# OHDSI/bayes-bridge

Measured on AMD Instinct MI355X. Metric: Gibbs iters/sec (cg sampler), higher is better.
Workload: dtype f64

## Files before the change

### bayes-bridge_amd/bayesbridge_amd/_lib.py

```python
import ctypes
import os
from ctypes import (POINTER, byref, c_char_p, c_double, c_int, c_int32,
                    c_int64, c_uint64, c_void_p)

_HERE = os.path.dirname(os.path.abspath(__file__))
LIB_PATH = os.path.join(os.path.dirname(_HERE), "libbbx.so")

ABI_VERSION = 113
FORMAT_AUTO, FORMAT_CSR, FORMAT_TILED = 0, 1, 2
F64, F32 = 0, 1
MODEL_LINEAR, MODEL_LOGIT = 0, 1
MODEL_PROBIT = 2
MODEL_STUDENT_T = 3
MODEL_CENSORED = 4
PRED_LINEAR, PRED_LOGIT, PRED_POISSON = 0, 1, 2
GSCALE_SAMPLE, GSCALE_OPTIMIZE, GSCALE_FIXED = 0, 1, 2
BATCH_ALLOW_SLOW = 1
ERR_NUMERIC = -4
COX_FAMILIES = ("cox", "coxcp", "coxef", "coxw", "coxfg")
SAMPLER_CG, SAMPLER_CHOLESKY, SAMPLER_WOODBURY = 0, 1, 2
STREAM_ETA1, STREAM_ETA2 = 1, 2

_lib = None
finalizing = False
# ... 131 lines not shown
        "bbx_chain_get_summary": (
            [hp, c_void_p, c_void_p, POINTER(c_int64)], c_int),
        "bbx_chain_init_obs_prec": ([hp], c_int),
        "bbx_chain_get_iteration": ([hp, POINTER(c_int64)], c_int),
        "bbx_chain_set_iteration": ([hp, c_int64], c_int),
        "bbx_chain_get_seed": ([hp, POINTER(c_uint64)], c_int),
        "bbx_chain_set_seed": ([hp, c_uint64], c_int),
        "bbx_chain_set_gscale_update": ([hp, c_int], c_int),
        "bbx_chain_set_coef_sampler": ([hp, c_int], c_int),
        "bbx_chol_release": ([hp], c_int),
        "bbx_chain_eta": ([hp, c_int64, c_void_p, c_void_p], c_int),
        "bbx_chain_get_logp": (
            [hp, POINTER(c_double), POINTER(c_double)], c_int),
        "bbx_chain_get_latent": ([hp, c_void_p], c_int),
        "bbx_chain_get_zbase": ([hp, c_void_p], c_int),
        "bbx_chain_set_df": ([hp, c_double], c_int),
        "bbx_chain_get_df": ([hp, POINTER(c_double)], c_int),
        "bbx_chain_run": (
            [hp, c_int, c_int, c_int, c_int, c_double, c_void_p, c_void_p,
             c_void_p, c_void_p, c_void_p, c_void_p], c_int),
        "bbx_chain_set_progress": ([hp, c_int, c_void_p, c_void_p], c_int),
        "bbx_chain_run_host": (
            [hp, c_int, c_int, c_int, c_int, c_double, c_void_p, c_void_p,
             c_void_p, c_void_p, c_void_p, c_void_p], c_int),
        "bbx_batch_create": ([hp, c_int, c_void_p, POINTER(hp)], c_int),
        "bbx_batch_create_opts": (
            [hp, c_int, c_void_p, ctypes.c_uint, POINTER(hp)], c_int),
        "bbx_batch_predict": ([hp, c_int, POINTER(c_double)], c_int),
        "bbx_batch_unconverged": ([hp, POINTER(c_int)], c_int),
        "bbx_batch_destroy": ([hp], c_int),
# ... 199 lines not shown
```

### bayes-bridge_amd/bayesbridge_amd/design_matrix.py

```python
import ctypes
import warnings
from ctypes import byref, c_double, c_int, c_int64, c_void_p

import numpy as np
import scipy.sparse as sparse

from . import _lib


def _ptr(a):
    return None if a is None else a.ctypes.data_as(c_void_p)


def remove_intercept_indicator(X):
    n_rows = X.shape[0]
    if sparse.issparse(X):
        first = np.asarray(X.mean(axis=0)).ravel()
        second = np.asarray(X.multiply(X).mean(axis=0)).ravel()
        variance = second - first ** 2
    else:
        variance = np.var(X, axis=0)
    constant = variance < n_rows * 2. ** -52
    if constant.any():
        warnings.warn(
# ... 84 lines not shown
        return (int(a.value), int(b.value)), (pa.value, pb.value)

    @property
    def cg_launches(self):
        from ctypes import c_int
        v = c_int()
        _lib.check(self._lib.bbx_design_cg_launches(self._h, byref(v)))
        return int(v.value)

    def cg_stats(self, reset=False):
        from ctypes import c_int64
        a, b, c = c_int64(), c_int64(), c_int64()
        _lib.check(self._lib.bbx_design_cg_stats(
            self._h, byref(a), byref(b), byref(c), 1 if reset else 0))
        return int(a.value), int(b.value), int(c.value)

    def set_cg_fold(self, on):
        _lib.check(self._lib.bbx_design_set_cg_fold(
            self._h, -1 if on is None else int(bool(on))))

    @property
    def fused_operator_bytes(self):
        v = c_int64()
        _lib.check(self._lib.bbx_design_fused_operator_bytes(self._h,
                                                              byref(v)))
        return int(v.value)

    def tiled_info(self, chains=1):
        out = {}
        base = {1: 0, 2: 2, 4: 4}[int(chains)]
# ... 331 lines not shown
```

### bayes-bridge_amd/bayesbridge_amd/device_chain.py

```python
from ctypes import byref, c_double, c_int64, c_uint64, c_void_p

import numpy as np

from . import _lib

_GSCALE_MODES = {'sample': _lib.GSCALE_SAMPLE, 'optimize': _lib.GSCALE_OPTIMIZE,
                 None: _lib.GSCALE_FIXED}


_MODEL_CODES = {'linear': _lib.MODEL_LINEAR, 'logit': _lib.MODEL_LOGIT,
                'probit': _lib.MODEL_PROBIT,
                'student_t': _lib.MODEL_STUDENT_T,
                'censored': _lib.MODEL_CENSORED}


def _ptr(a):
    return None if a is None else a.ctypes.data_as(c_void_p)


def _f64(a):
    return np.ascontiguousarray(a, dtype=np.float64)


class HipGibbsChain():
# ... 105 lines not shown
        df = float(df)
        if not (df > 0. and np.isfinite(df)):
            raise ValueError("df must be finite and positive: %r" % df)
        _lib.check(self._lib.bbx_chain_set_df(self._c, df))

    def get_df(self):
        df = c_double()
        _lib.check(self._lib.bbx_chain_get_df(self._c, byref(df)))
        return float(df.value)

    def get_zbase(self):
        out = np.empty(self.P)
        _lib.check(self._lib.bbx_chain_get_zbase(self._c, _ptr(out)))
        return out

    def init_obs_prec(self):
        _lib.check(self._lib.bbx_chain_init_obs_prec(self._c))

    def set_summary(self, mean, square, n_averaged):
        mean, square = _f64(mean), _f64(square)
        if mean.shape != (self.P,) or square.shape != (self.P,):
            raise ValueError("summaries must have length %d" % self.P)
        _lib.check(self._lib.bbx_chain_set_summary(
            self._c, _ptr(mean), _ptr(square), int(n_averaged)))

    def get_summary(self):
        mean, square, n_avg = np.empty(self.P), np.empty(self.P), c_int64()
        _lib.check(self._lib.bbx_chain_get_summary(
            self._c, _ptr(mean), _ptr(square), byref(n_avg)))
        return mean, square, int(n_avg.value)
# ... 197 lines not shown
```

### bayes-bridge_amd/csrc/api.hip

```cpp
#include <algorithm>
#include <cmath>
#include <cstring>
#include <new>

#include <fcntl.h>
#include <sys/file.h>
#include <unistd.h>

#include <condition_variable>
#include <mutex>
#include <thread>
#include <unordered_set>

#include "common.hpp"
#include "tiled_layout.hpp"

namespace bbx {

static thread_local std::string g_last_error;

void set_error(const std::string& msg) { g_last_error = msg; }
int fail(int code, const std::string& msg) {
  g_last_error = msg;
  return code;
// ... 1379 lines not shown

uint64_t bbx_launch_count(void) {
  return bbx::g_launch_count.load(std::memory_order_relaxed);
}

int bbx_design_cg_stats(bbx_design* h, int64_t* solves, int64_t* empty_launches,
                        int64_t* naps, int reset) {
  BBX_TRY(check_handle(h));
  if (solves) *solves = h->cg_solves;
  if (empty_launches) *empty_launches = h->cg_empty_launches;
  if (naps) *naps = h->cg_naps;
  if (reset) h->cg_solves = h->cg_empty_launches = h->cg_naps = 0;
  return BBX_OK;
}

int bbx_design_cg_launches(const bbx_design* h, int* per_iteration) {
  BBX_TRY(check_handle(h));
  if (!per_iteration) return fail(BBX_ERR_INVALID, "per_iteration is NULL");
  int n = 5;
  if (tiled_fold_applies(h)) {
    n = 3;
  } else if (!h->sparse && dense_fused_applies(h)) {
    n = 3;
  } else if (h->sparse && h->format == BBX_FORMAT_TILED) {
    int G = 0;
    if (!h->hybrid && tiled_describe(h, 0, nullptr, nullptr, nullptr, &G,
                                     nullptr, nullptr) == BBX_OK && G == 1)
      n = 4;
  }
  *per_iteration = n;
// ... 17 lines not shown
```

### bayes-bridge_amd/csrc/cg_sampler.hip

```cpp
#include <sys/prctl.h>
#include <time.h>

#include "common.hpp"
#include "philox.hpp"
#include "tiled_layout.hpp"

namespace bbx {

int launch_cg_setup(bbx_design* h, int n_unshrunk, const double* phi,
                    const double* sd, const double* x0, double* s, double* d,
                    double* xs, CGState* st, double atol);
int launch_cg_direction(bbx_design* h, int k, CGState* st,
                        const double* rr_part, const double* r, double* pvec,
                        const double* s, double* sp, double* c_part,
                        const double* d = nullptr, double* pdp_part = nullptr,
                        unsigned long long* word = nullptr,
                        unsigned long long tag = 0);
int launch_cg_update(bbx_design* h, int k, CGState* st, const double* pq_part,
                     const double* pvec, const double* q, double* x, double* r,
                     double* rr_part);
int launch_cg_finish(bbx_design* h, const double* s, const double* x,
                     double* coef);

__global__ __launch_bounds__(256) void fill_normal_kernel(
    int64_t len, uint64_t seed, uint64_t stream, double* __restrict__ out,
    int prio) {
  if (prio) __builtin_amdgcn_s_setprio(3);
  for (int64_t i = (int64_t)blockIdx.x * blockDim.x + threadIdx.x; i < len;
       i += (int64_t)gridDim.x * blockDim.x) {
    Philox g(seed, stream, (uint64_t)i);
    out[i] = g.normal();
  }
// ... 95 lines not shown
  double* sp = h->w_P[6].as<double>() + (h->intercept ? 1 : 0);
  CGState* st = h->cg_state.as<CGState>();
  const bool fold = tiled_fold_applies(h);
  double* sr = h->w_P[9].as<double>() + (h->intercept ? 1 : 0);
  double* tu = h->w_n[2].as<double>();

  if (d_eta1 == nullptr) {
    double* e1 = h->w_n[2].as<double>();
    double* e2 = h->w_P[8].as<double>();
    BBX_TRY(launch_fill_normal(h, h->n, seed, STREAM_ETA1, e1));
    BBX_TRY(launch_fill_normal(h, h->P, seed, STREAM_ETA2, e2));
    d_eta1 = e1;
    d_eta2 = e2;
  }

  BBX_TRY(launch_cg_setup(h, n_unshrunk, d_phi, d_sd, d_x0, s, d, x, st, atol));

  CGState* host_st = static_cast<CGState*>(h->host_pinned);
  if (x0_zero < 0) {
    int* d_flag = &st->pad;
    int* h_flag = reinterpret_cast<int*>(host_st);
    BBX_HIP(hipMemsetAsync(d_flag, 0, sizeof(int), h->stream));
    BBX_LAUNCH(any_nonzero_kernel, dim3(NPART), dim3(256), 0,
                       h->stream, h->P, d_x0, d_flag);
    BBX_HIP(hipGetLastError());
    BBX_HIP(hipMemcpyAsync(h_flag, d_flag, sizeof(int), hipMemcpyDeviceToHost,
                           h->stream));
    BBX_HIP(hipStreamSynchronize(h->stream));
    x0_zero = (*h_flag == 0) ? 1 : 0;
  }

// ... 1 lines not shown
    double* w = h->w_n[1].as<double>();
    TdotEpilogue ep;
    ep.mode = TD_RESID;
    ep.s = s;
    ep.d = d;
    ep.x = x0_zero ? nullptr : x;
    ep.z = d_z;
    ep.phi = d_phi;
    ep.eta2 = d_eta2;
    ep.dot_part = part_slot(h, PS_RR);
    if (fold) {
      ep.fold_sr = sr;
      ep.fold_cr_part = part_slot(h, PS_C);
    }
    if (!x0_zero && !h->sparse && dense_fused_applies(h)) {
      BBX_TRY(launch_prep_v(h, x, s, sp, part_slot(h, PS_C)));
      BBX_TRY(launch_sqrt_scale(h, d_omega, d_eta1, w, part_slot(h, PS_SUMW),
                                nullptr, true));
      const int st_f =
          launch_operator_dense_fused(h, sp, d_omega, ep, r, nullptr, w);
      if (st_f != 0)
        return st_f < 0 ? st_f
                        : fail(BBX_ERR_STATE,
                               "single-pass dense operator refused its design");
    } else {
      const double* t0 = nullptr;
      if (!x0_zero) {
        double* t = h->w_n[0].as<double>();
        BBX_TRY(launch_prep_v(h, x, s, sp, part_slot(h, PS_C)));
        BBX_TRY(launch_dot(h, sp, d_omega, t, nullptr));
        t0 = t;
      }
      BBX_TRY(launch_sqrt_scale(h, d_omega, d_eta1, w, part_slot(h, PS_SUMW),
                                t0, t0 == nullptr));
      BBX_TRY(launch_tdot(h, w, part_slot(h, PS_SUMW), ep, r));
    }
  }


  struct SkipScope {
    bbx_design* h;
    ~SkipScope() { h->skip_flag = nullptr; }
  } skip_scope{h};
  h->skip_flag = &st->done;
// ... 44 lines not shown
    ep.dot_part = part_slot(h, PS_RR);
    ep.cg_x = x;
    ep.cg_r = r;
    ep.cg_state = st;
    ep.cg_k = kk;
    ep.pdp_part = pdp;
    ep.twt_part = part_slot(h, PS_TWT);
    ep.fold_sr = sr;
    ep.fold_cr_part = part_slot(h, PS_C);
    BBX_TRY(launch_tdot(h, h->w_n[0].as<double>(), part_slot(h, PS_SUMW), ep, q));
    return timer_end(h, 2);
  };
  auto iteration = [&](int kk) -> int {
    if (fold) return folded_iteration(kk);
    BBX_TRY(launch_cg_direction(h, kk, st, part_slot(h, PS_RR), r, pvec, s, sp,
                                part_slot(h, PS_C), d, pdp, word, tag));
    return operator_and_update(kk);
  };
  static const int ahead_env = getenv("BBX_CG_AHEAD") ? atoi(getenv("BBX_CG_AHEAD")) : 0;
  const int ahead = ahead_env >= 1 ? (ahead_env < 64 ? ahead_env : 64)
                    : h->n >= 50000 ? 1 : h->n >= 10000 ? 2 : 4;
  int free_run = 0;
  if (h->cg_recent_n > 0) {
    free_run = h->cg_recent[0];
    for (int i = 1; i < h->cg_recent_n; ++i)
      free_run = h->cg_recent[i] < free_run ? h->cg_recent[i] : free_run;
    free_run -= 1;
  }
  if (free_run > maxiter) free_run = maxiter;
  static const int sleep_env = getenv("BBX_CG_SLEEP") ? atoi(getenv("BBX_CG_SLEEP")) : -1;
  static const bool sleep_on = sleep_env >= 0 ? sleep_env != 0 : cores_per_rank() < 3;
// ... 55 lines not shown
        h->cg_naps += 1;
      }
      slept = true;
      continue;
    }
    if (++spins > (1u << 14)) {
      const hipError_t qe = hipStreamQuery(h->stream);
      if (qe != hipSuccess && qe != hipErrorNotReady) BBX_HIP(qe);
      spins = 0;
    }
    __builtin_ia32_pause();
  }
  h->timer.cur_tag = -1;
  h->tail_ran = false;
  h->coef_in_flight = false;
  BBX_TRY(launch_cg_finish(h, s, x, d_coef));
  if (done) {
    if (!h->ev_poll)
      BBX_HIP(hipEventCreateWithFlags(&h->ev_poll, hipEventDisableTiming));
    BBX_HIP(hipEventRecord(h->ev_poll, h->stream));
    h->coef_in_flight = true;
    if (h->tail_hook) {
      const bool timing = h->timer.enabled;
      h->timer.enabled = false;
      h->skip_flag = nullptr;
      const int rc = h->tail_hook(h->tail_ctx);
      h->timer.enabled = timing;
      if (rc < 0) return rc;
      h->tail_ran = true;
    }
  } else {
// ... 32 lines not shown
```

### bayes-bridge_amd/csrc/chain.hip

```cpp
#include <cmath>
#include <new>
#include <string>
#include <vector>

#include "chain.hpp"
#include "philox.hpp"
#include "samplers.hpp"
#include "pg_queue.hpp"

namespace bbx {

__device__ inline double wsum(double x) { return wave_allsum(x); }

__device__ inline double block_total_256(double x) {
  __shared__ double s_w[256 / WAVE];
  x = wsum(x);
  if ((threadIdx.x & (WAVE - 1)) == 0) s_w[threadIdx.x / WAVE] = x;
  __syncthreads();
  double r = 0.;
  if (threadIdx.x == 0)
    for (int k = 0; k < 256 / WAVE; ++k) r += s_w[k];
  __syncthreads();
  return r;
}

__device__ inline double shrunk_scale(double gscale, double lscale,
                                      double slab) {
  const double raw = gscale * lscale;
  const double ratio = raw / slab;
  return raw / sqrt(1. + ratio * ratio);
}

__global__ __launch_bounds__(256) void chain_prior_kernel(
    int64_t P, int nu, int model, double slab, long long n_avg,
    const ChainScalars* __restrict__ sc, const double* __restrict__ lscale,
    const double* __restrict__ sd_unshrunk, const double* __restrict__ mean,
    const double* __restrict__ square, const double* __restrict__ zbase,
    double* __restrict__ phi, double* __restrict__ x0, double* __restrict__ sd,
    double* __restrict__ z, int store_idx, double* __restrict__ samp_gs,
    double* __restrict__ samp_lp) {
  const double g = sc->gscale;
  const double zs =
      (model == BBX_MODEL_LINEAR || model == BBX_MODEL_CENSORED) ? sc->obs_prec
                                                                 : 1.;
  if (store_idx >= 0 && blockIdx.x == 0 && threadIdx.x == 0) {
    samp_gs[store_idx] = g;
    samp_lp[store_idx] = sc->logp();
  }
  for (int64_t j = (int64_t)blockIdx.x * 256 + threadIdx.x; j < P;
       j += (int64_t)gridDim.x * 256) {
    double prior_sd, guess = mean[j];
    if (j < nu) {
      prior_sd = sd_unshrunk[j];
    } else {
      prior_sd = shrunk_scale(g, lscale[j - nu], slab);
      guess *= prior_sd;
    }
    phi[j] = 1. / prior_sd;
    x0[j] = guess;
    double est = 1.;
    if (n_avg > 1) {
      const double k = (double)n_avg;
      const double m = mean[j];
      const double var = k / (k - 1.) * (square[j] - m * m);
      const double w = (k - 1.) / (k - 1. + 5.);
      est = sqrt(w * var + (1. - w) * 1.);
    }
    sd[j] = est;
    z[j] = zs * zbase[j];
  }
}

#define BBX_BRANCH_PRIO() do { if (prio) __builtin_amdgcn_s_setprio(3); } while (0)
static int lscale_prio() {
  static const int on = getenv("BBX_LSCALE_PRIO") ? atoi(getenv("BBX_LSCALE_PRIO")) : 1;
  return on;
}
static int branch_prio() {
  static const int on = !(getenv("BBX_BRANCH_PRIO") && atoi(getenv("BBX_BRANCH_PRIO")) == 0);
  return on;
}
__global__ __launch_bounds__(256) void chain_summary_kernel(
    int64_t P, int nu, double slab, long long n_avg,
    const ChainScalars* __restrict__ sc, const double* __restrict__ lscale,
// ... 485 lines not shown
  if (!on || !h->sparse || h->format != BBX_FORMAT_TILED || h->hybrid) return false;
  int G = 0;
  return tiled_describe(h, 0, nullptr, nullptr, nullptr, &G, nullptr, nullptr) ==
             BBX_OK && G == 1;
}

static int chain_check(const bbx_chain* c) {
  if (!c || !c->h) return fail(BBX_ERR_INVALID, "chain handle is NULL");
  return BBX_OK;
}

static double power_exp_ave_magnitude(double exponent) {
  return std::tgamma(2. / exponent) / std::tgamma(1. / exponent);
}

int chain_pre_draw(bbx_chain* c) {
  bbx_design* h = c->h;
  hipStream_t s = h->stream;
  const int64_t P = h->P, n = h->n;
  ChainScalars* sc = c->scalars.as<ChainScalars>();
  BBX_LAUNCH(chain_prior_kernel, dim3(NPART), dim3(256), 0, s, P,
                     c->n_unshrunk, c->model, c->slab,
                     (long long)c->n_averaged, sc, c->lscale.as<double>(),
                     c->sd_unshrunk.as<double>(), c->mean.as<double>(),
                     c->square.as<double>(), c->zbase.as<double>(),
                     c->phi.as<double>(), c->x0.as<double>(),
                     c->sd.as<double>(), c->z.as<double>(), c->pending_store,
                     c->samp_gscale.as<double>(), c->samp_logp.as<double>());
  c->pending_store = -1;
  if (c->model == BBX_MODEL_LINEAR || c->model == BBX_MODEL_CENSORED)
    BBX_LAUNCH(chain_fill_obs_prec_kernel, dim3(grid_for(n, ROW_GRID)),
                       dim3(256), 0, s, n, sc, c->obs_prec.as<double>());
  BBX_HIP(hipGetLastError());
  return BBX_OK;
}

int chain_post_draw(bbx_chain* c, bool have_psi, int phases,
                    bbx_chain* branch_of) {
  bbx_design* h = c->h;
  hipStream_t s = h->stream;
  const int64_t P = h->P, n = h->n;
  const int nu = c->n_unshrunk;
  const int64_t n_shrunk = P - nu;
  ChainScalars* sc = c->scalars.as<ChainScalars>();
// ... 112 lines not shown

  launch_err = hipGetLastError();
  if (phases & POST_JOIN) {
    if (fork) {
      BBX_HIP(hipEventRecord(c->ev_join, s_b));
      BBX_HIP(hipStreamWaitEvent(s, c->ev_join, 0));
    }
    c->iter += 1;
  }
  BBX_HIP(launch_err);
  return BBX_OK;
}

static int chain_step(bbx_chain* c, int maxiter, double atol, int* n_cg_iter) {
  const uint64_t it = (uint64_t)c->iter;
  BBX_TRY(chain_pre_draw(c));
  int info = 0;
  const bool have_eta = c->eta_iter == (long long)it && c->eta1_next.ptr;
  if (c->coef_sampler == BBX_SAMPLER_CHOLESKY) {
    bbx_design* h = c->h;
    if (!have_eta) {
      if (!c->eta2_next.ptr)
        BBX_TRY(c->eta2_next.alloc(sizeof(double) * (size_t)h->P));
      BBX_TRY(launch_fill_normal(h, h->P, cg_draw_seed(c, it), STREAM_ETA2,
                                 c->eta2_next.as<double>()));
    }
    const bool linear = c->model == BBX_MODEL_LINEAR ||
                        c->model == BBX_MODEL_CENSORED;
    const bool probit = c->model == BBX_MODEL_PROBIT;
    const int st = chol_sample_device(
        h, linear || probit ? nullptr : c->obs_prec.as<double>(), 1.,
// ... 32 lines not shown
        linear || probit ? 0 : 1, c->eta1_next.as<double>(), c->eta2_next.as<double>(),
        c->coef.as<double>());
    c->eta_iter = -1;
    if (st < 0) return st;
    c->coef_sample = nullptr;
    if (n_cg_iter) *n_cg_iter = 0;
    BBX_TRY(chain_post_draw(c, false, POST_ALL));
    return 0;
  }
  struct TailScope {
    bbx_design* h;
    ~TailScope() {
      h->tail_hook = nullptr;
      h->tail_ctx = nullptr;
      h->coef_copy = nullptr;
    }
  } tail_scope{c->h};
  c->h->coef_copy = c->coef_sample;
  if (chain_tail_applies(c)) {
    c->h->tail_hook = chain_tail_hook;
    c->h->tail_ctx = c;
  }

  int st = cg_sample_device(
      c->h, c->obs_prec.as<double>(), c->phi.as<double>(), c->z.as<double>(),
      c->x0.as<double>(), c->sd.as<double>(), c->n_unshrunk,
      have_eta ? c->eta1_next.as<double>() : nullptr,
      have_eta ? c->eta2_next.as<double>() : nullptr,
      cg_draw_seed(c, it), maxiter, atol, c->coef.as<double>(), n_cg_iter,
      &info, c->mean_zero ? 1 : 0);
  c->eta_iter = -1;
  if (st < 0) return st;
  c->mean_zero = false;
// ... 500 lines not shown
      return fail(BBX_ERR_INVALID, "bbx_chain_get_df: not a student_t chain");
    if (!df) return fail(BBX_ERR_INVALID, "bbx_chain_get_df: df is NULL");
    *df = c->df;
    return BBX_OK;
  });
}

int bbx_chain_get_zbase(bbx_chain* c, double* out) {
  return no_throw([&]() -> int {
    BBX_TRY(chain_check(c));
    if (!out) return fail(BBX_ERR_INVALID, "bbx_chain_get_zbase: out is NULL");
    BBX_HIP(hipSetDevice(c->h->device));
    BBX_HIP(hipStreamSynchronize(c->h->stream));
    BBX_HIP(hipMemcpy(out, c->zbase.ptr, sizeof(double) * (size_t)c->h->P,
                      hipMemcpyDeviceToHost));
    return BBX_OK;
  });
}

int bbx_chain_init_obs_prec(bbx_chain* c) {
  BBX_TRY(chain_check(c));
  bbx_design* h = c->h;
  BBX_HIP(hipSetDevice(h->device));
  if (c->model == BBX_MODEL_PROBIT) return chain_probit_refresh(c);
  BBX_TRY(chain_linear_predictor(c));
  const int rg = grid_for(h->n, ROW_GRID);
  if (c->model == BBX_MODEL_STUDENT_T) {
    double* rp = c->row_part.as<double>();
    BBX_LAUNCH(chain_rss_kernel, dim3(rg), dim3(256), 0, h->stream, h->n,
               c->outcome.as<double>(), c->psi.as<double>(), rp);
// ... 302 lines not shown
```

### bayes-bridge_amd/csrc/chain.hpp

```cpp
#pragma once
#include <cmath>

#include "common.hpp"

namespace bbx {

constexpr int ROW_GRID = 2048;

struct alignas(128) ChainScalars {
  double gscale;
  double logprior;
  double abs_pow_sum;
  long long n_gscale_clamped;
  long long n_lscale_fixed;
  alignas(128) double obs_prec;
  double loglik;
  __host__ __device__ double logp() const { return loglik + logprior; }
};

}

struct bbx_chain {
  bbx_design* h = nullptr;
  int model = BBX_MODEL_LOGIT;
// ... 23 lines not shown
  long long eta_iter = -1;
  bbx::DevMem samp_gscale, samp_logp;
  int pending_store = -1;
  double* coef_sample = nullptr;
  void* pinned = nullptr;
  hipStream_t stream2 = nullptr;
  hipEvent_t ev_join = nullptr;
};

namespace bbx {

inline uint64_t cg_draw_seed(const bbx_chain* c, uint64_t it) {
  return c->seed + 0x9E3779B97F4A7C15ull * (it + 1);
}

int chain_pre_draw(bbx_chain* c);
enum { POST_BRANCH = 1, POST_MAIN = 2, POST_JOIN = 4, POST_ALL = 7 };
int chain_post_draw(bbx_chain* c, bool have_psi, int phases,
                    bbx_chain* branch_of = nullptr);
int chain_begin_run(bbx_chain* c, int n_sample);
int chain_save_sample(bbx_chain* c, int idx, double* d_coef, double* d_lscale,
                      double* d_obs_prec);
int chain_end_run(bbx_chain* c, int n_sample, double* gscale, double* logp);

int launch_chain_probit(bbx_chain* c, uint64_t stream, int* row_blocks);
int launch_sumw_fold(bbx_design* h, const double* block_sums, int count);

int launch_student_t_tau(bbx_chain* c, uint64_t stream);
int launch_student_t_mix(bbx_chain* c, uint64_t stream, int* row_blocks);
int launch_student_t_finish(bbx_chain* c, int row_blocks);
double student_t_row_const(double nu);
// ... 5 lines not shown
```

### bayes-bridge_amd/csrc/common.hpp

```cpp
#pragma once

#include <hip/hip_runtime.h>
#include <stdint.h>

#include <exception>
#include <new>
#include <string>
#include <vector>

#include "../../include/bbx.h"

#include <atomic>
namespace bbx {
extern std::atomic<unsigned long long> g_launch_count;
}
#define BBX_LAUNCH(...)                                                   \
  do {                                                                    \
    bbx::g_launch_count.fetch_add(1, std::memory_order_relaxed);          \
    hipLaunchKernelGGL(__VA_ARGS__);                                      \
  } while (0)
#define BBX_LAUNCH_EXT(...)                                               \
  do {                                                                    \
    bbx::g_launch_count.fetch_add(1, std::memory_order_relaxed);          \
    hipExtLaunchKernelGGL(__VA_ARGS__);                                   \
// ... 97 lines not shown
  }
};

struct CGState {
  double rho[2];
  double atol;
  double bnorm2;
  int n_iter;
  int done;
  int bad;
  int pad;
  int running;
  int pad2;
};

struct KernelTimer {
  bool enabled = false;
  int period = 1;
  static constexpr int FAMILIES = 3;
  int64_t seen[FAMILIES] = {0, 0, 0};
  bool armed[FAMILIES] = {false, false, false};
  struct Pair {
    hipEvent_t a, b;
    int tag;
  };
  std::vector<Pair> pending[FAMILIES];
  std::vector<Pair> pool;
  int cur_tag = -1;
  std::vector<float> samples[FAMILIES];
};
// ... 50 lines not shown

  int64_t n_dot = 0, n_tdot = 0;
  int last_cg_iter = 0;
  unsigned long long* cg_word_host = nullptr;
  unsigned long long* cg_word_dev = nullptr;
  unsigned long long cg_serial = 0;
  int cg_recent[8] = {0, 0, 0, 0, 0, 0, 0, 0};
  int cg_recent_n = 0;
  int64_t cg_period_ns = 0;
  bool coef_in_flight = false;
  int64_t cg_empty_launches = 0, cg_solves = 0, cg_naps = 0;
  double* coef_copy = nullptr;
  int (*tail_hook)(void*) = nullptr;
  void* tail_ctx = nullptr;
  bool tail_ran = false;
  hipEvent_t ev_poll = nullptr;
  bool in_operator = false;
  uint64_t operator_serial = 0;
  int cg_fold = -1;
  const int* skip_flag = nullptr;
  bbx::KernelTimer timer;
};

namespace bbx {

enum PartSlot {
  PS_C = 0,
  PS_SUMW = 1,
  PS_PQ = 2,
  PS_RR = 3,
// ... 204 lines not shown
```

### bayes-bridge_amd/csrc/vecops.hip

```cpp
#include "common.hpp"

namespace bbx {

std::atomic<unsigned long long> g_launch_count{0};


__device__ inline double wave_sum_v(double x) { return wave_allsum(x); }

__device__ inline void block_store_partial(double x, double* part) {
  __shared__ double s_w[VEC_BLOCK / WAVE];
  x = wave_sum_v(x);
  if ((threadIdx.x & (WAVE - 1)) == 0) s_w[threadIdx.x / WAVE] = x;
  __syncthreads();
  if (threadIdx.x == 0) {
    double r = 0.;
#pragma unroll
    for (int k = 0; k < VEC_BLOCK / WAVE; ++k) r += s_w[k];
    part[blockIdx.x] = r;
  }
  __syncthreads();
}

__device__ inline double sum_partials_v(const double* part) {
  __shared__ double s_tot;
// ... 127 lines not shown
    const double sj = (jj < n_unshrunk) ? 2. * sd[jj] : 1. / ph;
    const double sp = sj * ph;
    s[jj] = sj;
    d[jj] = sp * sp;
    xs[jj] = x0[jj] / sj;
  }
}

__global__ __launch_bounds__(VEC_BLOCK) void cg_direction_kernel(
    int64_t P, int intercept, int k, CGState* __restrict__ st,
    const double* __restrict__ rr_part, const double* __restrict__ r,
    double* __restrict__ pvec, const double* __restrict__ s,
    const double* __restrict__ offset, double* __restrict__ sp,
    double* __restrict__ c_part, const double* __restrict__ d,
    double* __restrict__ pdp_part, unsigned long long* word,
    unsigned long long tag) {
  const PartLoad pl = part_issue(rr_part);
  const int64_t stride = (int64_t)gridDim.x * VEC_BLOCK;
  const int64_t j0 = (int64_t)blockIdx.x * VEC_BLOCK + threadIdx.x;
  const bool has0 = j0 < P;
  double r0 = 0., p0 = 0., s0 = 0., o0 = 0., d0 = 0.;
  if (has0) {
    r0 = r[j0];
    if (k > 0) p0 = pvec[j0];
    s0 = s[j0];
    if (j0 >= intercept) o0 = offset[j0 - intercept];
    if (pdp_part) d0 = d[j0];
  }
  const int was_done = st->done;
  const double atol = st->atol;
  const double rho_prev = (k > 0) ? st->rho[(k - 1) & 1] : 1.;
  if (was_done) return;
  const double rho = part_finish(pl);
  const bool finite = (rho == rho) && (rho - rho == 0.);
  if (!finite || sqrt(rho) < atol) {
    if (blockIdx.x == 0 && threadIdx.x == 0) {
      st->done = 1;
      st->running = 0;
      if (!finite) st->bad = 1;
      if (word)
        cg_word_store(word, tag | CG_WORD_DONE | (finite ? 0ull : CG_WORD_BAD) |
                                (unsigned long long)k);
    }
    return;
  }
  if (word && blockIdx.x == 0 && threadIdx.x == 0)
    cg_word_store(word, tag | (unsigned long long)(k + 1));
  const double beta = (k > 0) ? rho / rho_prev : 0.;
  double acc = 0., acc_d = 0.;
  if (has0) {
    double pj = r0;
    if (k > 0) pj += beta * p0;
    pvec[j0] = pj;
    const double v = s0 * pj;
    sp[j0] = v;
    if (j0 >= intercept) acc += o0 * v;
    acc_d += d0 * pj * pj;
// ... 63 lines not shown

int launch_cg_setup(bbx_design* h, int n_unshrunk, const double* phi,
                    const double* sd, const double* x0, double* s, double* d,
                    double* xs, CGState* st, double atol) {
  BBX_LAUNCH(cg_setup_kernel, dim3(NPART), dim3(VEC_BLOCK), 0,
                     h->stream, h->P, n_unshrunk, phi, sd, x0, s, d, xs, st,
                     atol);
  BBX_HIP(hipGetLastError());
  return BBX_OK;
}

int launch_cg_direction(bbx_design* h, int k, CGState* st,
                        const double* rr_part, const double* r, double* pvec,
                        const double* s, double* sp, double* c_part,
                        const double* d, double* pdp_part,
                        unsigned long long* word, unsigned long long tag) {
  BBX_LAUNCH(cg_direction_kernel, dim3(NPART), dim3(VEC_BLOCK), 0,
                     h->stream, h->P, h->intercept, k, st, rr_part, r, pvec, s,
                     h->offset.as<double>(), sp, c_part, d, pdp_part, word, tag);
  BBX_HIP(hipGetLastError());
  return BBX_OK;
}

int launch_cg_update(bbx_design* h, int k, CGState* st, const double* pq_part,
                     const double* pvec, const double* q, double* x, double* r,
                     double* rr_part) {
  BBX_LAUNCH(cg_update_kernel, dim3(NPART), dim3(VEC_BLOCK), 0,
                     h->stream, h->P, k, st, pq_part, pvec, q, x, r, rr_part);
  BBX_HIP(hipGetLastError());
  return BBX_OK;
}

int launch_cg_finish(bbx_design* h, const double* s, const double* x,
                     double* coef) {
// ... 8 lines not shown
```

### include/bbx.h

```cpp
#ifndef BBX_H
#define BBX_H

#include <stdint.h>

#ifdef __cplusplus
extern "C" {
#endif

#define BBX_VERSION 113

#define BBX_OK 0
#define BBX_ERR_INVALID (-1)
#define BBX_ERR_HIP (-2)
#define BBX_ERR_NODEVICE (-3)
#define BBX_ERR_NUMERIC (-4)
#define BBX_ERR_STATE (-5)

#define BBX_FORMAT_AUTO 0
#define BBX_FORMAT_CSR 1
#define BBX_FORMAT_TILED 2

#define BBX_F64 0
#define BBX_F32 1

// ... 53 lines not shown
int bbx_design_is_sparse(const bbx_design* h, int* flag);
int bbx_design_is_binary(const bbx_design* h, int* flag);
int bbx_design_device(const bbx_design* h, int* device);
int bbx_design_format(const bbx_design* h, int* format);
int bbx_design_storage_bytes(const bbx_design* h, int64_t* bytes);
int bbx_design_matvec_bytes(const bbx_design* h, int64_t* dot_bytes,
                            int64_t* tdot_bytes);
int bbx_design_timed_bytes(const bbx_design* h, int64_t* dot_bytes,
                           int64_t* tdot_bytes);
int bbx_design_useful_bytes(const bbx_design* h, int64_t* dot_bytes,
                            int64_t* tdot_bytes, double* pad_dot,
                            double* pad_tdot);
int bbx_design_cg_launches(const bbx_design* h, int* per_iteration);
int bbx_design_cg_stats(bbx_design* h, int64_t* solves, int64_t* empty_launches,
                        int64_t* naps, int reset);
uint64_t bbx_launch_count(void);
int bbx_design_set_cg_fold(bbx_design* h, int on);
int bbx_design_fused_operator_bytes(const bbx_design* h, int64_t* bytes);

int bbx_design_hybrid_info(const bbx_design* h, int* is_hybrid,
                           int64_t* ones_nnz, int64_t* rest_nnz,
                           int64_t* dense_nnz, int* dense_cols);
enum {
  BBX_HYB_DOT_NONE = 0,
  BBX_HYB_DOT_EPI = 1,
  BBX_HYB_DOT_FUSED_WAVE = 2,
  BBX_HYB_DOT_FUSED_WG = 3,
  BBX_HYB_DOT_SEPARATE = 4,
  BBX_HYB_DOT_SEPARATE_SLABS = 5
};
// ... 110 lines not shown
int bbx_chain_get_iteration(bbx_chain* c, int64_t* iteration);
int bbx_chain_set_iteration(bbx_chain* c, int64_t iteration);
int bbx_chain_get_seed(bbx_chain* c, uint64_t* seed);
int bbx_chain_set_seed(bbx_chain* c, uint64_t seed);
int bbx_chain_set_gscale_update(bbx_chain* c, int mode);
#define BBX_SAMPLER_CG 0
#define BBX_SAMPLER_CHOLESKY 1
#define BBX_SAMPLER_WOODBURY 2
int bbx_chain_set_coef_sampler(bbx_chain* c, int sampler);
int bbx_chain_eta(bbx_chain* c, int64_t iteration, double* eta1, double* eta2);
int bbx_chain_get_logp(bbx_chain* c, double* loglik, double* logp);
int bbx_chain_get_latent(bbx_chain* c, double* out);
int bbx_chain_set_df(bbx_chain* c, double df);
int bbx_chain_get_df(bbx_chain* c, double* df);
int bbx_chain_get_zbase(bbx_chain* c, double* out);

int bbx_chain_run(bbx_chain* c, int n_iter, int n_burnin, int thin,
                  int maxiter, double atol, double* d_coef, double* d_lscale,
                  double* d_obs_prec, double* gscale, double* logp,
                  double* n_cg_iter);
int bbx_chain_set_progress(bbx_chain* c, int every, void (*fn)(int, void*),
                           void* ctx);
int bbx_chain_run_host(bbx_chain* c, int n_iter, int n_burnin, int thin,
                       int maxiter, double atol, double* coef, double* lscale,
                       double* obs_prec, double* gscale, double* logp,
                       double* n_cg_iter);

int bbx_batch_create(bbx_design* design, int n_chain, bbx_chain* const* chains,
                     bbx_batch** out);
#define BBX_BATCH_ALLOW_SLOW 1u
// ... 518 lines not shown
```

Before: 329.6.

## Fuse chain prior kernel into CG setup and fold finish into direction kernel

The per-iteration prior kernel (phi, x0, sd, z) is merged with the CG set-up and warm-start prep_v work into one kernel, invoked through a new setup hook on the design. Separately, the CG direction kernel now writes coef = s*x (and the coef copy) when it detects convergence, so the separate finish launch is skipped in the non-folded path when the solve converged. Both aim to cut kernel launches and extra passes over P-length vectors per Gibbs iteration. Debug APIs are added to read back the set-up vectors and CG state for comparison.

```diff
diff --git a/bayes-bridge_amd/bayesbridge_amd/_lib.py b/bayes-bridge_amd/bayesbridge_amd/_lib.py
--- a/bayes-bridge_amd/bayesbridge_amd/_lib.py
+++ b/bayes-bridge_amd/bayesbridge_amd/_lib.py
@@ -169,6 +169,10 @@
             [hp, POINTER(c_double), POINTER(c_double)], c_int),
         "bbx_chain_get_latent": ([hp, c_void_p], c_int),
         "bbx_chain_get_zbase": ([hp, c_void_p], c_int),
+        "bbx_chain_cg_setup": (
+            [hp, c_int, c_int, c_double, c_void_p, c_void_p, c_void_p], c_int),
+        "bbx_design_cg_vectors": (
+            [hp, c_void_p, c_void_p, c_void_p, c_void_p, c_void_p], c_int),
         "bbx_chain_set_df": ([hp, c_double], c_int),
         "bbx_chain_get_df": ([hp, POINTER(c_double)], c_int),
         "bbx_chain_run": (
diff --git a/bayes-bridge_amd/bayesbridge_amd/design_matrix.py b/bayes-bridge_amd/bayesbridge_amd/design_matrix.py
--- a/bayes-bridge_amd/bayesbridge_amd/design_matrix.py
+++ b/bayes-bridge_amd/bayesbridge_amd/design_matrix.py
@@ -122,6 +122,16 @@
         _lib.check(self._lib.bbx_design_cg_stats(
             self._h, byref(a), byref(b), byref(c), 1 if reset else 0))
         return int(a.value), int(b.value), int(c.value)
+
+    def cg_vectors(self):
+        import numpy as np
+        P = self.shape[1]
+        out = {k: np.empty(P) for k in ('s', 'd', 'x', 'r')}
+        out['state'] = np.empty(10)
+        _lib.check(self._lib.bbx_design_cg_vectors(
+            self._h, *(out[k].ctypes.data for k in ('s', 'd', 'x', 'r',
+                                                    'state'))))
+        return out
 
     def set_cg_fold(self, on):
         _lib.check(self._lib.bbx_design_set_cg_fold(
diff --git a/bayes-bridge_amd/bayesbridge_amd/device_chain.py b/bayes-bridge_amd/bayesbridge_amd/device_chain.py
--- a/bayes-bridge_amd/bayesbridge_amd/device_chain.py
+++ b/bayes-bridge_amd/bayesbridge_amd/device_chain.py
@@ -143,6 +143,16 @@
         _lib.check(self._lib.bbx_chain_get_zbase(self._c, _ptr(out)))
         return out
 
+    def cg_setup(self, fused, warm, atol):
+        vecs = np.empty((8, self.P))
+        c_part, state = np.empty(256), np.empty(10)
+        _lib.check(self._lib.bbx_chain_cg_setup(
+            self._c, int(bool(fused)), int(bool(warm)), float(atol),
+            _ptr(vecs), _ptr(c_part), _ptr(state)))
+        out = dict(zip(('phi', 'x0', 'sd', 'z', 's', 'd', 'xs', 'sp'), vecs))
+        out['c_part'], out['state'] = c_part, state
+        return out
+
     def init_obs_prec(self):
         _lib.check(self._lib.bbx_chain_init_obs_prec(self._c))
 
diff --git a/bayes-bridge_amd/csrc/api.hip b/bayes-bridge_amd/csrc/api.hip
--- a/bayes-bridge_amd/csrc/api.hip
+++ b/bayes-bridge_amd/csrc/api.hip
@@ -1417,6 +1417,40 @@
   return BBX_OK;
 }
 
+static void cg_state_doubles(const CGState& st, double* out) {
+  out[0] = st.rho[0];
+  out[1] = st.rho[1];
+  out[2] = st.atol;
+  out[3] = st.bnorm2;
+  out[4] = st.n_iter;
+  out[5] = st.done;
+  out[6] = st.bad;
+  out[7] = st.pad;
+  out[8] = st.running;
+  out[9] = st.pad2;
+}
+
+int bbx_design_cg_vectors(bbx_design* h, double* s, double* d, double* x,
+                          double* r, double* state) {
+  return no_throw([&]() -> int {
+    BBX_TRY(check_handle(h));
+    BBX_HIP(hipSetDevice(h->device));
+    BBX_HIP(hipStreamSynchronize(h->stream));
+    double* const out[4] = {s, d, x, r};
+    for (int i = 0; i < 4; ++i)
+      if (out[i])
+        BBX_HIP(hipMemcpy(out[i], h->w_P[i].ptr, sizeof(double) * (size_t)h->P,
+                          hipMemcpyDeviceToHost));
+    if (state) {
+      CGState st;
+      BBX_HIP(hipMemcpy(&st, h->cg_state.ptr, sizeof(CGState),
+                        hipMemcpyDeviceToHost));
+      cg_state_doubles(st, state);
+    }
+    return BBX_OK;
+  });
+}
+
 int bbx_design_cg_launches(const bbx_design* h, int* per_iteration) {
   BBX_TRY(check_handle(h));
   if (!per_iteration) return fail(BBX_ERR_INVALID, "per_iteration is NULL");
diff --git a/bayes-bridge_amd/csrc/cg_sampler.hip b/bayes-bridge_amd/csrc/cg_sampler.hip
--- a/bayes-bridge_amd/csrc/cg_sampler.hip
+++ b/bayes-bridge_amd/csrc/cg_sampler.hip
@@ -15,7 +15,8 @@
                         const double* s, double* sp, double* c_part,
                         const double* d = nullptr, double* pdp_part = nullptr,
                         unsigned long long* word = nullptr,
-                        unsigned long long tag = 0);
+                        unsigned long long tag = 0, const double* x = nullptr,
+                        double* coef = nullptr);
 int launch_cg_update(bbx_design* h, int k, CGState* st, const double* pq_part,
                      const double* pvec, const double* q, double* x, double* r,
                      double* rr_part);
@@ -141,7 +142,14 @@
     d_eta2 = e2;
   }
 
-  BBX_TRY(launch_cg_setup(h, n_unshrunk, d_phi, d_sd, d_x0, s, d, x, st, atol));
+  const bool fused_setup = h->setup_hook != nullptr && x0_zero >= 0;
+  if (fused_setup) {
+    const CGSetup su{n_unshrunk, s, d, x, st, atol, x0_zero ? nullptr : sp,
+                     part_slot(h, PS_C)};
+    BBX_TRY(h->setup_hook(h->setup_ctx, su));
+  } else {
+    BBX_TRY(launch_cg_setup(h, n_unshrunk, d_phi, d_sd, d_x0, s, d, x, st, atol));
+  }
 
   CGState* host_st = static_cast<CGState*>(h->host_pinned);
   if (x0_zero < 0) {
@@ -173,7 +181,7 @@
       ep.fold_cr_part = part_slot(h, PS_C);
     }
     if (!x0_zero && !h->sparse && dense_fused_applies(h)) {
-      BBX_TRY(launch_prep_v(h, x, s, sp, part_slot(h, PS_C)));
+      if (!fused_setup) BBX_TRY(launch_prep_v(h, x, s, sp, part_slot(h, PS_C)));
       BBX_TRY(launch_sqrt_scale(h, d_omega, d_eta1, w, part_slot(h, PS_SUMW),
                                 nullptr, true));
       const int st_f =
@@ -186,7 +194,7 @@
       const double* t0 = nullptr;
       if (!x0_zero) {
         double* t = h->w_n[0].as<double>();
-        BBX_TRY(launch_prep_v(h, x, s, sp, part_slot(h, PS_C)));
+        if (!fused_setup) BBX_TRY(launch_prep_v(h, x, s, sp, part_slot(h, PS_C)));
         BBX_TRY(launch_dot(h, sp, d_omega, t, nullptr));
         t0 = t;
       }
@@ -261,7 +269,8 @@
   auto iteration = [&](int kk) -> int {
     if (fold) return folded_iteration(kk);
     BBX_TRY(launch_cg_direction(h, kk, st, part_slot(h, PS_RR), r, pvec, s, sp,
-                                part_slot(h, PS_C), d, pdp, word, tag));
+                                part_slot(h, PS_C), d, pdp, word, tag, x,
+                                d_coef));
     return operator_and_update(kk);
   };
   static const int ahead_env = getenv("BBX_CG_AHEAD") ? atoi(getenv("BBX_CG_AHEAD")) : 0;
@@ -347,7 +356,7 @@
   h->timer.cur_tag = -1;
   h->tail_ran = false;
   h->coef_in_flight = false;
-  BBX_TRY(launch_cg_finish(h, s, x, d_coef));
+  if (!done || fold) BBX_TRY(launch_cg_finish(h, s, x, d_coef));
   if (done) {
     if (!h->ev_poll)
       BBX_HIP(hipEventCreateWithFlags(&h->ev_poll, hipEventDisableTiming));
diff --git a/bayes-bridge_amd/csrc/chain.hip b/bayes-bridge_amd/csrc/chain.hip
--- a/bayes-bridge_amd/csrc/chain.hip
+++ b/bayes-bridge_amd/csrc/chain.hip
@@ -9,6 +9,10 @@
 #include "pg_queue.hpp"
 
 namespace bbx {
+
+int launch_cg_setup(bbx_design* h, int n_unshrunk, const double* phi,
+                    const double* sd, const double* x0, double* s, double* d,
+                    double* xs, CGState* st, double atol);
 
 __device__ inline double wsum(double x) { return wave_allsum(x); }
 
@@ -29,6 +33,37 @@
   const double raw = gscale * lscale;
   const double ratio = raw / slab;
   return raw / sqrt(1. + ratio * ratio);
+}
+
+struct PriorTerms {
+  double phi, x0, sd, z;
+};
+__device__ __forceinline__ PriorTerms prior_terms(
+    int64_t j, int nu, double slab, long long n_avg, double g, double zs,
+    const double* __restrict__ lscale, const double* __restrict__ sd_unshrunk,
+    const double* __restrict__ mean, const double* __restrict__ square,
+    const double* __restrict__ zbase) {
+  double prior_sd, guess = mean[j];
+  if (j < nu) {
+    prior_sd = sd_unshrunk[j];
+  } else {
+    prior_sd = shrunk_scale(g, lscale[j - nu], slab);
+    guess *= prior_sd;
+  }
+  PriorTerms t;
+  t.phi = 1. / prior_sd;
+  t.x0 = guess;
+  double est = 1.;
+  if (n_avg > 1) {
+    const double k = (double)n_avg;
+    const double m = mean[j];
+    const double var = k / (k - 1.) * (square[j] - m * m);
+    const double w = (k - 1.) / (k - 1. + 5.);
+    est = sqrt(w * var + (1. - w) * 1.);
+  }
+  t.sd = est;
+  t.z = zs * zbase[j];
+  return t;
 }
 
 __global__ __launch_bounds__(256) void chain_prior_kernel(
@@ -49,25 +84,71 @@
   }
   for (int64_t j = (int64_t)blockIdx.x * 256 + threadIdx.x; j < P;
        j += (int64_t)gridDim.x * 256) {
-    double prior_sd, guess = mean[j];
-    if (j < nu) {
-      prior_sd = sd_unshrunk[j];
-    } else {
-      prior_sd = shrunk_scale(g, lscale[j - nu], slab);
-      guess *= prior_sd;
-    }
-    phi[j] = 1. / prior_sd;
-    x0[j] = guess;
-    double est = 1.;
-    if (n_avg > 1) {
-      const double k = (double)n_avg;
-      const double m = mean[j];
-      const double var = k / (k - 1.) * (square[j] - m * m);
-      const double w = (k - 1.) / (k - 1. + 5.);
-      est = sqrt(w * var + (1. - w) * 1.);
-    }
-    sd[j] = est;
-    z[j] = zs * zbase[j];
+    const PriorTerms t = prior_terms(j, nu, slab, n_avg, g, zs, lscale,
+                                     sd_unshrunk, mean, square, zbase);
+    phi[j] = t.phi;
+    x0[j] = t.x0;
+    sd[j] = t.sd;
+    z[j] = t.z;
+  }
+}
+
+__global__ __launch_bounds__(256) void chain_prior_setup_kernel(
+    int64_t P, int nu, int model, double slab, long long n_avg,
+    const ChainScalars* __restrict__ sc, const double* __restrict__ lscale,
+    const double* __restrict__ sd_unshrunk, const double* __restrict__ mean,
+    const double* __restrict__ square, const double* __restrict__ zbase,
+    double* __restrict__ phi, double* __restrict__ x0, double* __restrict__ sd,
+    double* __restrict__ z, int store_idx, double* __restrict__ samp_gs,
+    double* __restrict__ samp_lp, int intercept,
+    const double* __restrict__ offset, double* __restrict__ s,
+    double* __restrict__ d, double* __restrict__ xs, CGState* __restrict__ st,
+    double atol, double* __restrict__ sp, double* __restrict__ c_part) {
+  const double g = sc->gscale;
+  const double zs =
+      (model == BBX_MODEL_LINEAR || model == BBX_MODEL_CENSORED) ? sc->obs_prec
+                                                                 : 1.;
+  if (blockIdx.x == 0 && threadIdx.x == 0) {
+    if (store_idx >= 0) {
+      samp_gs[store_idx] = g;
+      samp_lp[store_idx] = sc->logp();
+    }
+    st->rho[0] = st->rho[1] = 0.;
+    st->atol = atol;
+    st->bnorm2 = 0.;
+    st->n_iter = 0;
+    st->done = 0;
+    st->bad = 0;
+    st->pad = 0;
+    st->running = 1;
+    st->pad2 = 0;
+  }
+  double acc = 0.;
+  for (int64_t j = (int64_t)blockIdx.x * 256 + threadIdx.x; j < P;
+       j += (int64_t)gridDim.x * 256) {
+    const PriorTerms t = prior_terms(j, nu, slab, n_avg, g, zs, lscale,
+                                     sd_unshrunk, mean, square, zbase);
+    phi[j] = t.phi;
+    x0[j] = t.x0;
+    sd[j] = t.sd;
+    z[j] = t.z;
+    const double ph = t.phi;
+    const double sj = (j < nu) ? 2. * t.sd : 1. / ph;
+    const double sph = sj * ph;
+    s[j] = sj;
+    d[j] = sph * sph;
+    const double xsj = t.x0 / sj;
+    xs[j] = xsj;
+    if (sp) {
+      double val = xsj;
+      val *= sj;
+      sp[j] = val;
+      if (j >= intercept) acc += offset[j - intercept] * val;
+    }
+  }
+  if (sp) {
+    const double tot = block_total_256(acc);
+    if (threadIdx.x == 0) c_part[blockIdx.x] = tot;
   }
 }
 
@@ -583,20 +664,46 @@
   return std::tgamma(2. / exponent) / std::tgamma(1. / exponent);
 }
 
-int chain_pre_draw(bbx_chain* c) {
+static int launch_chain_prior(bbx_chain* c, const CGSetup* su) {
+  bbx_design* h = c->h;
+  ChainScalars* sc = c->scalars.as<ChainScalars>();
+  if (su)
+    BBX_LAUNCH(chain_prior_setup_kernel, dim3(NPART), dim3(256), 0, h->stream,
+               h->P, c->n_unshrunk, c->model, c->slab,
+               (long long)c->n_averaged, sc, c->lscale.as<double>(),
+               c->sd_unshrunk.as<double>(), c->mean.as<double>(),
+               c->square.as<double>(), c->zbase.as<double>(),
+               c->phi.as<double>(), c->x0.as<double>(), c->sd.as<double>(),
+               c->z.as<double>(), c->pending_store,
+               c->samp_gscale.as<double>(), c->samp_logp.as<double>(),
+               h->intercept, h->offset.as<double>(), su->s, su->d, su->xs,
+               su->st, su->atol, su->sp, su->c_part);
+  else
+    BBX_LAUNCH(chain_prior_kernel, dim3(NPART), dim3(256), 0, h->stream, h->P,
+               c->n_unshrunk, c->model, c->slab, (long long)c->n_averaged, sc,
+               c->lscale.as<double>(), c->sd_unshrunk.as<double>(),
+               c->mean.as<double>(), c->square.as<double>(),
+               c->zbase.as<double>(), c->phi.as<double>(), c->x0.as<double>(),
+               c->sd.as<double>(), c->z.as<double>(), c->pending_store,
+               c->samp_gscale.as<double>(), c->samp_logp.as<double>());
+  c->pending_store = -1;
+  BBX_HIP(hipGetLastError());
+  return BBX_OK;
+}
+
+static int chain_setup_hook(void* ctx, const CGSetup& su) {
+  bbx_chain* c = static_cast<bbx_chain*>(ctx);
+  if (su.n_unshrunk != c->n_unshrunk)
+    return fail(BBX_ERR_STATE, "fused set-up: n_unshrunk is not the chain's");
+  return launch_chain_prior(c, &su);
+}
+
+int chain_pre_draw(bbx_chain* c, bool prior_in_setup) {
   bbx_design* h = c->h;
   hipStream_t s = h->stream;
-  const int64_t P = h->P, n = h->n;
+  const int64_t n = h->n;
   ChainScalars* sc = c->scalars.as<ChainScalars>();
-  BBX_LAUNCH(chain_prior_kernel, dim3(NPART), dim3(256), 0, s, P,
-                     c->n_unshrunk, c->model, c->slab,
-                     (long long)c->n_averaged, sc, c->lscale.as<double>(),
-                     c->sd_unshrunk.as<double>(), c->mean.as<double>(),
-                     c->square.as<double>(), c->zbase.as<double>(),
-                     c->phi.as<double>(), c->x0.as<double>(),
-                     c->sd.as<double>(), c->z.as<double>(), c->pending_store,
-                     c->samp_gscale.as<double>(), c->samp_logp.as<double>());
-  c->pending_store = -1;
+  if (!prior_in_setup) BBX_TRY(launch_chain_prior(c, nullptr));
   if (c->model == BBX_MODEL_LINEAR || c->model == BBX_MODEL_CENSORED)
     BBX_LAUNCH(chain_fill_obs_prec_kernel, dim3(grid_for(n, ROW_GRID)),
                        dim3(256), 0, s, n, sc, c->obs_prec.as<double>());
@@ -739,7 +846,7 @@
 
 static int chain_step(bbx_chain* c, int maxiter, double atol, int* n_cg_iter) {
   const uint64_t it = (uint64_t)c->iter;
-  BBX_TRY(chain_pre_draw(c));
+  BBX_TRY(chain_pre_draw(c, c->coef_sampler == BBX_SAMPLER_CG));
   int info = 0;
   const bool have_eta = c->eta_iter == (long long)it && c->eta1_next.ptr;
   if (c->coef_sampler == BBX_SAMPLER_CHOLESKY) {
@@ -802,9 +909,13 @@
       h->tail_hook = nullptr;
       h->tail_ctx = nullptr;
       h->coef_copy = nullptr;
+      h->setup_hook = nullptr;
+      h->setup_ctx = nullptr;
     }
   } tail_scope{c->h};
   c->h->coef_copy = c->coef_sample;
+  c->h->setup_hook = chain_setup_hook;
+  c->h->setup_ctx = c;
   if (chain_tail_applies(c)) {
     c->h->tail_hook = chain_tail_hook;
     c->h->tail_ctx = c;
@@ -1335,6 +1446,55 @@
     BBX_HIP(hipStreamSynchronize(c->h->stream));
     BBX_HIP(hipMemcpy(out, c->zbase.ptr, sizeof(double) * (size_t)c->h->P,
                       hipMemcpyDeviceToHost));
+    return BBX_OK;
+  });
+}
+
+int bbx_chain_cg_setup(bbx_chain* c, int fused, int warm, double atol,
+                       double* vecs, double* c_part, double* state) {
+  return no_throw([&]() -> int {
+    BBX_TRY(chain_check(c));
+    if (!vecs || !c_part || !state)
+      return fail(BBX_ERR_INVALID, "bbx_chain_cg_setup: an output is NULL");
+    bbx_design* h = c->h;
+    const size_t P = (size_t)h->P;
+    BBX_HIP(hipSetDevice(h->device));
+    double* s = h->w_P[0].as<double>();
+    double* d = h->w_P[1].as<double>();
+    double* xs = h->w_P[2].as<double>();
+    double* sp = h->w_P[6].as<double>() + (h->intercept ? 1 : 0);
+    CGState* st = h->cg_state.as<CGState>();
+    double* cp = part_slot(h, PS_C);
+    BBX_HIP(hipMemsetAsync(st, 0xFF, sizeof(CGState), h->stream));
+    BBX_HIP(hipMemsetAsync(sp, 0, sizeof(double) * P, h->stream));
+    BBX_HIP(hipMemsetAsync(cp, 0, sizeof(double) * NPART, h->stream));
+    const int pending = c->pending_store;
+    c->pending_store = -1;
+    const CGSetup su{c->n_unshrunk, s, d, xs, st, atol, warm ? sp : nullptr, cp};
+    int rc = launch_chain_prior(c, fused ? &su : nullptr);
+    c->pending_store = pending;
+    BBX_TRY(rc);
+    if (!fused) {
+      BBX_TRY(launch_cg_setup(h, c->n_unshrunk, c->phi.as<double>(),
+                              c->sd.as<double>(), c->x0.as<double>(), s, d, xs,
+                              st, atol));
+      if (warm) BBX_TRY(launch_prep_v(h, xs, s, sp, cp));
+    }
+    BBX_HIP(hipStreamSynchronize(h->stream));
+    const void* src[8] = {c->phi.ptr, c->x0.ptr, c->sd.ptr, c->z.ptr,
+                          s, d, xs, sp};
+    for (int i = 0; i < 8; ++i)
+      BBX_HIP(hipMemcpy(vecs + (size_t)i * P, src[i], sizeof(double) * P,
+                        hipMemcpyDeviceToHost));
+    BBX_HIP(hipMemcpy(c_part, cp, sizeof(double) * NPART,
+                      hipMemcpyDeviceToHost));
+    CGState hst;
+    BBX_HIP(hipMemcpy(&hst, st, sizeof(CGState), hipMemcpyDeviceToHost));
+    const double out[10] = {hst.rho[0], hst.rho[1], hst.atol, hst.bnorm2,
+                            (double)hst.n_iter, (double)hst.done,
+                            (double)hst.bad, (double)hst.pad,
+                            (double)hst.running, (double)hst.pad2};
+    for (int i = 0; i < 10; ++i) state[i] = out[i];
     return BBX_OK;
   });
 }
diff --git a/bayes-bridge_amd/csrc/chain.hpp b/bayes-bridge_amd/csrc/chain.hpp
--- a/bayes-bridge_amd/csrc/chain.hpp
+++ b/bayes-bridge_amd/csrc/chain.hpp
@@ -61,7 +61,7 @@
   return c->seed + 0x9E3779B97F4A7C15ull * (it + 1);
 }
 
-int chain_pre_draw(bbx_chain* c);
+int chain_pre_draw(bbx_chain* c, bool prior_in_setup = false);
 enum { POST_BRANCH = 1, POST_MAIN = 2, POST_JOIN = 4, POST_ALL = 7 };
 int chain_post_draw(bbx_chain* c, bool have_psi, int phases,
                     bbx_chain* branch_of = nullptr);
diff --git a/bayes-bridge_amd/csrc/common.hpp b/bayes-bridge_amd/csrc/common.hpp
--- a/bayes-bridge_amd/csrc/common.hpp
+++ b/bayes-bridge_amd/csrc/common.hpp
@@ -135,6 +135,17 @@
   int pad2;
 };
 
+struct CGSetup {
+  int n_unshrunk;
+  double* s;
+  double* d;
+  double* xs;
+  CGState* st;
+  double atol;
+  double* sp;
+  double* c_part;
+};
+
 struct KernelTimer {
   bool enabled = false;
   int period = 1;
@@ -215,6 +226,8 @@
   int (*tail_hook)(void*) = nullptr;
   void* tail_ctx = nullptr;
   bool tail_ran = false;
+  int (*setup_hook)(void*, const bbx::CGSetup&) = nullptr;
+  void* setup_ctx = nullptr;
   hipEvent_t ev_poll = nullptr;
   bool in_operator = false;
   uint64_t operator_serial = 0;
diff --git a/bayes-bridge_amd/csrc/vecops.hip b/bayes-bridge_amd/csrc/vecops.hip
--- a/bayes-bridge_amd/csrc/vecops.hip
+++ b/bayes-bridge_amd/csrc/vecops.hip
@@ -165,7 +165,8 @@
     const double* __restrict__ offset, double* __restrict__ sp,
     double* __restrict__ c_part, const double* __restrict__ d,
     double* __restrict__ pdp_part, unsigned long long* word,
-    unsigned long long tag) {
+    unsigned long long tag, const double* __restrict__ x,
+    double* __restrict__ coef, double* __restrict__ copy) {
   const PartLoad pl = part_issue(rr_part);
   const int64_t stride = (int64_t)gridDim.x * VEC_BLOCK;
   const int64_t j0 = (int64_t)blockIdx.x * VEC_BLOCK + threadIdx.x;
@@ -179,9 +180,10 @@
     if (pdp_part) d0 = d[j0];
   }
   const int was_done = st->done;
+  const int n_iter = st->n_iter;
   const double atol = st->atol;
   const double rho_prev = (k > 0) ? st->rho[(k - 1) & 1] : 1.;
-  if (was_done) return;
+  if (was_done && !(coef && n_iter == k)) return;
   const double rho = part_finish(pl);
   const bool finite = (rho == rho) && (rho - rho == 0.);
   if (!finite || sqrt(rho) < atol) {
@@ -192,6 +194,13 @@
       if (word)
         cg_word_store(word, tag | CG_WORD_DONE | (finite ? 0ull : CG_WORD_BAD) |
                                 (unsigned long long)k);
+    }
+    if (coef) {
+      for (int64_t jj = j0; jj < P; jj += stride) {
+        const double v = s[jj] * x[jj];
+        coef[jj] = v;
+        if (copy) copy[jj] = v;
+      }
     }
     return;
   }
@@ -285,10 +294,12 @@
                         const double* rr_part, const double* r, double* pvec,
                         const double* s, double* sp, double* c_part,
                         const double* d, double* pdp_part,
-                        unsigned long long* word, unsigned long long tag) {
+                        unsigned long long* word, unsigned long long tag,
+                        const double* x, double* coef) {
   BBX_LAUNCH(cg_direction_kernel, dim3(NPART), dim3(VEC_BLOCK), 0,
                      h->stream, h->P, h->intercept, k, st, rr_part, r, pvec, s,
-                     h->offset.as<double>(), sp, c_part, d, pdp_part, word, tag);
+                     h->offset.as<double>(), sp, c_part, d, pdp_part, word, tag,
+                     x, coef, coef ? h->coef_copy : nullptr);
   BBX_HIP(hipGetLastError());
   return BBX_OK;
 }
diff --git a/include/bbx.h b/include/bbx.h
--- a/include/bbx.h
+++ b/include/bbx.h
@@ -91,6 +91,8 @@
 int bbx_design_cg_launches(const bbx_design* h, int* per_iteration);
 int bbx_design_cg_stats(bbx_design* h, int64_t* solves, int64_t* empty_launches,
                         int64_t* naps, int reset);
+int bbx_design_cg_vectors(bbx_design* h, double* s, double* d, double* x,
+                          double* r, double* state);
 uint64_t bbx_launch_count(void);
 int bbx_design_set_cg_fold(bbx_design* h, int on);
 int bbx_design_fused_operator_bytes(const bbx_design* h, int64_t* bytes);
@@ -231,6 +233,8 @@
 int bbx_chain_set_df(bbx_chain* c, double df);
 int bbx_chain_get_df(bbx_chain* c, double* df);
 int bbx_chain_get_zbase(bbx_chain* c, double* out);
+int bbx_chain_cg_setup(bbx_chain* c, int fused, int warm, double atol,
+                       double* vecs, double* c_part, double* state);
 
 int bbx_chain_run(bbx_chain* c, int n_iter, int n_burnin, int thin,
                   int maxiter, double atol, double* d_coef, double* d_lscale,
```

Measured after the change: 328.0. Within noise of the previous version (-0.5%).
